# Amar-Aliaga/Stereo_Depth_Ruler

Measured on AMD Instinct MI355X. Metric: stereo Mpix/s (disparity+reproject) at 1280×720 d=128, 1/2/4/8 MI355X, higher is better.
Workload: dtype int16; 1 GPU; C2 (BASELINE configs[1]): 1280x720 d=128 MODE_SGBM 5-path + reprojectImageTo3D(Q, handleMissing), batch 1; width=1280, height=720, numDisparities=128, mode=MODE_SGBM, batch=1, pipeline=sgbm, parallelism=frame shard x1, streams_per_gpu=2

## Files before the change

stereo_depth_ruler_amd/csrc/sdr_device.hpp:

```cpp
#pragma once
#include <hip/hip_runtime.h>
#include <cfloat>
#include <stdint.h>

#include <type_traits>
#include <utility>

namespace sdr {

typedef short s16x2 __attribute__((ext_vector_type(2)));

constexpr int kMaxCost = 32767;
constexpr uint32_t kMaxPair = 0x7fff7fffu;

__device__ __forceinline__ s16x2 as_s16x2(uint32_t v) { return __builtin_bit_cast(s16x2, v); }
__device__ __forceinline__ uint32_t as_u32(s16x2 v) { return __builtin_bit_cast(uint32_t, v); }

__device__ __forceinline__ uint32_t pk_add(uint32_t a, uint32_t b) {
    return as_u32(as_s16x2(a) + as_s16x2(b));
}
__device__ __forceinline__ uint32_t pk_sub(uint32_t a, uint32_t b) {
    return as_u32(as_s16x2(a) - as_s16x2(b));
}
__device__ __forceinline__ uint32_t pk_add_sat(uint32_t a, uint32_t b) {
// ... 80 lines not shown
    uint32_t t = (uint32_t)__builtin_amdgcn_update_dpp((int)0xffffffff, (int)m, 0x142, 0xa, 0xf, false);
    m = min(m, t);
    t = (uint32_t)__builtin_amdgcn_update_dpp((int)0xffffffff, (int)m, 0x143, 0xc, 0xf, false);
    m = min(m, t);
    return (uint32_t)__builtin_amdgcn_readlane((int)m, 63);
}

__device__ __forceinline__ uint32_t row16_min_u32(uint32_t m) {
    m = min_u32_dpp<kDppQuadXor1>(m);
    m = min_u32_dpp<kDppQuadXor2>(m);
    m = min_u32_dpp<kDppRowHalfMirror>(m);
    return min_u32_dpp<kDppRowMirror>(m);
}

template <int K>
struct Regs {
    uint32_t r[K];
};

using Rsrc = __amdgpu_buffer_rsrc_t;
__device__ __forceinline__ Rsrc rsrc_at(const void* base) {
    return __builtin_amdgcn_make_buffer_rsrc(const_cast<void*>(base), (short)0, 0x7fffffff, 0x00020000);
}

template <int K, int AUX = 0>
__device__ __forceinline__ Regs<K> load_buf(Rsrc r, uint32_t vofs, uint32_t sofs = 0) {
    Regs<K> v;
    if constexpr (K == 1) {
        v.r[0] = __builtin_amdgcn_raw_buffer_load_b32(r, vofs, sofs, AUX);
    } else if constexpr (K == 2) {
        const auto t = __builtin_amdgcn_raw_buffer_load_b64(r, vofs, sofs, AUX);
        v.r[0] = t[0];
        v.r[1] = t[1];
    } else {
        static_assert(K % 4 == 0, "K = 1, 2 or a multiple of 4");
#pragma unroll
        for (int j = 0; j < K / 4; j++) {
            const auto t = __builtin_amdgcn_raw_buffer_load_b128(r, vofs + 16 * j, sofs, AUX);
            v.r[4 * j] = t[0]; v.r[4 * j + 1] = t[1]; v.r[4 * j + 2] = t[2]; v.r[4 * j + 3] = t[3];
        }
    }
    return v;
}

template <int K, int AUX = 2>
__device__ __forceinline__ void store_buf_nt(Rsrc r, uint32_t vofs, uint32_t sofs, const Regs<K>& v) {
    if constexpr (K == 1) {
        __builtin_amdgcn_raw_buffer_store_b32(v.r[0], r, vofs, sofs, AUX);
    } else if constexpr (K == 2) {
        __builtin_amdgcn_raw_buffer_store_b64((__attribute__((ext_vector_type(2))) uint32_t){v.r[0], v.r[1]}, r,
                                              vofs, sofs, AUX);
    } else {
#pragma unroll
        for (int j = 0; j < K / 4; j++)
            __builtin_amdgcn_raw_buffer_store_b128(
                (__attribute__((ext_vector_type(4))) uint32_t){v.r[4 * j], v.r[4 * j + 1], v.r[4 * j + 2],
                                                               v.r[4 * j + 3]},
                r, vofs + 16 * j, sofs, AUX);
    }
}

__device__ __forceinline__ int lane_id() { return (int)__lane_id(); }

inline int device_cus() {
    static int cache[64] = {};
    int dev = 0;
    (void)hipGetDevice(&dev);
    if (dev < 0 || dev >= 64) dev = 0;
    int cus = __atomic_load_n(&cache[dev], __ATOMIC_RELAXED);
    if (cus <= 0) {
        if (hipDeviceGetAttribute(&cus, hipDeviceAttributeMultiprocessorCount, dev) != hipSuccess || cus <= 0) cus = 256;
        __atomic_store_n(&cache[dev], cus, __ATOMIC_RELAXED);
    }
    return cus;
}

__device__ __forceinline__ int xcd_block(int h, int n) {
    const int q = n >> 3, r = n & 7, x = h & 7, k = h >> 3;
    return (x < r ? x * (q + 1) : r * (q + 1) + (x - r) * q) + k;
}

template <typename F, int... J>
__device__ __forceinline__ void unroll_rows(F& f, int k0, std::integer_sequence<int, J...>) {
    (f(k0 + J, std::integral_constant<int, J>{}), ...);
}
template <typename F, int... J>
__device__ __forceinline__ void unroll_rows_tail(F& f, int k0, int klast, std::integer_sequence<int, J...>) {
    ((k0 + J <= klast ? f(k0 + J, std::integral_constant<int, J>{}) : void()), ...);
}

__device__ __forceinline__ int div_trunc_small(int n, int d) {
    const int an = abs(n);
// ... 38 lines not shown
```

stereo_depth_ruler_amd/csrc/sdr_engine.hip:

```cpp
#include "../../include/sdr/sdr.h"
#include "sdr_internal.hpp"

#include <hip/hip_runtime.h>

#include <algorithm>
#include <cmath>
#include <cstdio>
#include <cstring>
#include <map>
#include <mutex>
#include <string>
#include <vector>

namespace {

thread_local std::string g_last_error;

int fail(int code, const std::string& msg) {
    g_last_error = msg;
    return code;
}

#define SDR_HIP(call)                                                                    \
    do {                                                                                 \
        hipError_t e_ = (call);                                                          \
        if (e_ != hipSuccess)                                                            \
            return fail(SDR_ERR_DEVICE, std::string(#call) + ": " + hipGetErrorString(e_)); \
    } while (0)

struct Eff {
    sdr::Geometry g;
    int mode, uniq, uniq_simd, disp12MaxDiff, ftzero, nstripes, invalid;
    int speckle_ws, speckle_diff, blockSize;
    int cost;
};

int make_eff(const sdr_sgbm_params& p, int W, int H, Eff* e, int cost = SDR_COST_BT) {
    if (cost != SDR_COST_BT && cost != SDR_COST_CENSUS_9X7) return fail(SDR_ERR_ARG, "unknown cost type");
    e->cost = cost;
    if (p.numDisparities <= 0 || p.numDisparities % 16 != 0)
// ... 267 lines not shown
    int drain() {
        for (const Out& o : outs) {
            SDR_HIP(hipEventSynchronize(ev[o.ev]));
            if (!o.dst) continue;
            if (o.dpitch == o.rowbytes) std::memcpy(o.dst, o.src, o.rowbytes * o.rows);
            else
                for (int r = 0; r < o.rows; r++) std::memcpy(o.dst + r * o.dpitch, o.src + r * o.rowbytes, o.rowbytes);
        }
        outs.clear();
        return SDR_OK;
    }
    void release() {
        for (auto e : ev) (void)hipEventDestroy(e);
        ev.clear();
        if (pin) (void)hipHostFree(pin);
        pin = nullptr;
        cap = 0;
    }
};
size_t stage_bytes(size_t n) { return (n + 255) & ~(size_t)255; }
}

struct sdr_sgbm {
    sdr_sgbm_params p{};
    int cost = SDR_COST_BT;
    size_t census_bytes = 0;
    int device = 0;
    hipStream_t stream = nullptr;
    hipStream_t own_stream = nullptr;
    Buf planesL, planesR, sink, C, Lr, Caux, draw, dlr, dfin, labels, sizes, mins, hin, hxyz, keys2;
    Buf sweep, status;
    int* status_host = nullptr;
    int sweep_spin = sdr::kSweepSpin;
    HostXfer hx;
    Buf cls_bgr, cls_gray, cls_small, cls_dl, cls_wls, cls_f, cls_conf, cls_filt;
    int timing = 0;
    hipEvent_t ev[4] = {nullptr, nullptr, nullptr, nullptr};
    std::vector<hipEvent_t> kev;
    std::vector<int> kkind;
    size_t kused = 0;
    size_t path_slack = 0, path_lslack = 0;
    hipStream_t side = nullptr;
    hipEvent_t fork = nullptr, join = nullptr;
    hipEvent_t done = nullptr;
    bool pending = false;
    bool persistent = true;
    bool relayed = false;
    bool needs_wait = false;
    int status_reported = 0;
    bool lr_skipped = false;
    sdr::Geometry lr_g{};
    int lr_frames = 0, lr_d12 = 0;
    size_t aux_slack = 0;
};

namespace {
constexpr unsigned kOrderEvent = hipEventDisableTiming | hipEventReleaseToDevice;
constexpr unsigned kTimerEvent = hipEventReleaseToDevice;
bool capturing(hipStream_t s) {
    hipStreamCaptureStatus cs = hipStreamCaptureStatusNone;
    return hipStreamIsCapturing(s, &cs) == hipSuccess && cs == hipStreamCaptureStatusActive;
}
hipError_t relay(sdr_sgbm* h, hipStream_t from) {
    hipError_t e = hipEventRecord(h->done, from);
    if (e == hipSuccess) e = hipStreamWaitEvent(h->own_stream, h->done, 0);
    if (e == hipSuccess) e = hipEventRecord(h->done, h->own_stream);
// ... 298 lines not shown
                d.Caux = Caux + s * (size_t)amax * g.W1 * g.D;
                d.aux_row0 = sp.s0;
                d.aux_rows = sp.aux_rows;
            }
        }
    } else if (e.mode == SDR_MODE_HH4) {
        add_dir(plS, sdr::DIR_S, nS, nullptr);
        add_dir(pls, sdr::DIR_N, nS, buf());
    } else if (sweep) {
    } else {
        add_dir(plS, sdr::DIR_S, nS, nullptr);
        if (e.mode == SDR_MODE_HH) add_dir(pls, sdr::DIR_N, nS, buf());
        add_dir(pls, sdr::DIR_SE, nD, buf());
        add_dir(pls, sdr::DIR_SW, nD, buf());
        if (e.mode == SDR_MODE_HH) {
            add_dir(pls, sdr::DIR_NE, nD, buf());
            add_dir(pls, sdr::DIR_NW, nD, buf());
        }
    }
    for (size_t s = 0; s < stripes.size(); s++) {
        const Stripe& sp = stripes[s];
        if (sp.aux_rows == 0 || sp.aux_rows != sp.end - sp.s0 || sp.out0 >= sp.end) continue;
        if (pls.nredir == sdr::kMaxCostAux) return fail(SDR_ERR_ARG, "too many 3WAY stripes");
        sdr::RowRedirect& r = pls.redir[pls.nredir++];
        r.lo = sp.out0;
        r.hi = sp.end;
        r.s0 = sp.s0;
        r.aux = Caux + s * (size_t)amax * g.W1 * g.D;
    }
    for (sdr::PathLaunch* pl : {&pls, &plS}) {
        pl->prefix[0] = 0;
        for (int i = 0; i < pl->ndirs; i++) pl->prefix[i + 1] = pl->prefix[i] + pl->d[i].nchains;
    }
    { KTimer kt(h, SDR_KERNEL_PATHS); sdr::launch_paths(g, pls, F, st); }
    if (sweep) {
        char* sb = (char*)h->sweep.p;
        SDR_HIP(hipMemsetAsync(sb, 0, sweep_flags + sizeof(int), st));
        sdr::SweepArgs sa{};
        sa.C = C;
        sa.cs_fstride = cells;
        sa.l_fstride = lfs;
        sa.l_pix = nrec * g.D;
        sa.flags = (int*)sb;
        sa.err = (int*)(sb + sweep_flags);
        sa.edge = (uint32_t*)(sb + sweep_flags + 256);
        sa.spin = h->sweep_spin;
        sdr::SweepWta sw{};
        sw.recs = Lr;
        sw.disp_raw = draw;
        sw.d2 = d2;
        sw.disp_fstride = px;
        sw.uniq = e.uniq;
        sw.uniq_simd = e.uniq_simd;
        std::lock_guard<std::mutex> lk(g_sweep_mu);
        hipEvent_t& last = g_sweep_last[h->device];
        if (last) SDR_HIP(hipStreamWaitEvent(st, last, 0));
        else SDR_HIP(hipEventCreateWithFlags(&last, kOrderEvent));
        for (int up = 1; up >= 0; up--) {
            sa.up = up;
            sa.ntiles = shp[up].ntiles;
            sa.nslots = shp[up].nslots;
            sa.rec = Lr + (size_t)2 * g.D;
            KTimer kt(h, up ? SDR_KERNEL_SWEEP : SDR_KERNEL_SWEEP_DOWN);
            sdr::launch_sweep(g, sa, sw, F, st);
            sa.flags += flags_n[up];
        }
// ... 52 lines not shown
    p->blockSize = 3;
    p->mode = SDR_MODE_SGBM;
    p->nstripes = 4;
}

void sdr_right_matcher_params(const sdr_sgbm_params* l, sdr_sgbm_params* r) {
    if (!l || !r) return;
    sdr_sgbm_params_default(r);
    r->minDisparity = -(l->minDisparity + l->numDisparities) + 1;
    r->numDisparities = l->numDisparities;
    r->blockSize = l->blockSize;
    r->uniquenessRatio = 0;
    r->P1 = l->P1;
    r->P2 = l->P2;
    r->mode = l->mode;
    r->preFilterCap = l->preFilterCap;
    r->disp12MaxDiff = 1000000;
    r->speckleWindowSize = 0;
    r->speckleRange = l->speckleRange;
    r->nstripes = l->nstripes;
    r->uniq_rule = l->uniq_rule;
}

int sdr_sgbm_create(const sdr_sgbm_params* p, int device, sdr_sgbm** out) {
    if (!p || !out) return fail(SDR_ERR_ARG, "null argument");
    *out = nullptr;
    int ndev = 0;
    SDR_HIP(hipGetDeviceCount(&ndev));
    if (device < 0 || device >= ndev) return fail(SDR_ERR_DEVICE, "invalid device index");
    SDR_HIP(hipSetDevice(device));
    sdr_sgbm* h = new sdr_sgbm();
    h->p = *p;
    h->device = device;
    if (hipStreamCreateWithFlags(&h->own_stream, hipStreamNonBlocking) != hipSuccess) {
        delete h;
        return fail(SDR_ERR_DEVICE, "hipStreamCreate failed");
    }
    h->stream = h->own_stream;
    for (auto& ev : h->ev) (void)hipEventCreateWithFlags(&ev, kTimerEvent);
    (void)hipEventCreateWithFlags(&h->done, kOrderEvent);
    *out = h;
    return SDR_OK;
}

int sdr_sgbm_destroy(sdr_sgbm* h) {
    if (!h) return SDR_OK;
    (void)hipSetDevice(h->device);
    if (h->stream && h->persistent) (void)hipStreamSynchronize(h->stream);
    if (h->own_stream && h->own_stream != h->stream) (void)hipStreamSynchronize(h->own_stream);
    if (h->status_host) (void)hipHostFree(h->status_host);
    for (Buf* b : {&h->sweep, &h->status, &h->planesL, &h->planesR, &h->sink, &h->C, &h->Lr, &h->Caux, &h->draw, &h->dlr, &h->dfin, &h->keys2,
                   &h->labels, &h->sizes, &h->mins, &h->hin, &h->hxyz, &h->cls_bgr,
                   &h->cls_gray, &h->cls_small, &h->cls_dl, &h->cls_wls, &h->cls_f,
                   &h->cls_conf, &h->cls_filt})
        if (b->p) (void)hipFree(b->p);
    h->hx.release();
    for (auto ev : h->ev)
        if (ev) (void)hipEventDestroy(ev);
    for (auto ev : h->kev) (void)hipEventDestroy(ev);
    if (h->side) (void)hipStreamSynchronize(h->side);
    if (h->fork) (void)hipEventDestroy(h->fork);
    if (h->join) (void)hipEventDestroy(h->join);
    if (h->done) (void)hipEventDestroy(h->done);
    if (h->side) (void)hipStreamDestroy(h->side);
    if (h->own_stream) (void)hipStreamDestroy(h->own_stream);
    delete h;
// ... 600 lines not shown
```

stereo_depth_ruler_amd/csrc/sdr_internal.hpp:

```cpp
#pragma once
#include <hip/hip_runtime.h>

#include "../../include/sdr/sdr.h"
#include <stddef.h>
#include <stdint.h>

#include <string>

namespace sdr {

constexpr int kMinSlots = 256;


struct Buf {
    void* p = nullptr;
    size_t n = 0;
};
int ensure(Buf& b, size_t bytes);
hipError_t scratch_alloc(void** p, size_t bytes, hipStream_t st);
hipError_t scratch_free(void* p, hipStream_t st);
int set_error(int code, const std::string& msg);

enum Dir : int {
    DIR_E = 0,
// ... 48 lines not shown
    int ylim;
    int hh_bottom;
    int TY;
    int16_t* sink;
    int naux;
    size_t aux_fstride;
    CostAux aux[kMaxCostAux];
};
size_t cost_sink_bytes(const Geometry& g);


constexpr int kMaxPathDirs = 24;
constexpr int kMaxPaths = 8;

struct PathDir {
    int dir;
    int nchains;
    int ybeg, yend, write_from;
    int aux_row0, aux_rows;
    const int16_t* Caux;
    int16_t* out;
};

struct RowRedirect {
    int lo, hi, s0;
    const int16_t* aux;
};

struct PathLaunch {
    const int16_t* C;
    size_t cs_fstride;
    size_t l_fstride;
    int l_pix;
    size_t aux_fstride;
    int ndirs;
    int prefix[kMaxPathDirs + 1];
    PathDir d[kMaxPathDirs];
    int nredir;
    RowRedirect redir[kMaxCostAux];
};

constexpr int kSweepOwn = 10;
constexpr int kSweepWaves = kSweepOwn + 2;
struct SweepArgs {
    const int16_t* C;
    size_t cs_fstride;
    int16_t* rec;
    size_t l_fstride;
    int l_pix;
    uint32_t* edge;
    int* flags;
    int* err;
    int ntiles, nslots;
    int up;
    int spin;
    int xcd;
};
struct SweepWta {
    const int16_t* recs;
    int16_t* disp_raw;
    uint32_t* d2;
    size_t disp_fstride;
    int uniq, uniq_simd;
};
constexpr int kSweepSpin = 1 << 20;
void launch_sweep_verdict(const int* err, int16_t* disp, size_t n, int F, int16_t invalid, int* mins,
                          int* sticky, hipStream_t st);
struct SweepShape {
    int cols, ntiles, nslots, npub, entry_words;
};
SweepShape sweep_shape(const Geometry& g, int F, bool up);
void launch_sweep(const Geometry& g, const SweepArgs& a, const SweepWta& w, int F, hipStream_t st);

constexpr int kSouthIdx = 2;
constexpr int kSouthPad = 64;
struct SouthWtaArgs {
    const int16_t* L;
    int npaths;
    int16_t* disp_raw;
    uint32_t* d2;
    size_t disp_fstride;
    int uniq, uniq_simd;
};
void launch_south_wta(const Geometry& g, const PathLaunch& pl, const SouthWtaArgs& a, int F,
                      hipStream_t st);

constexpr uint32_t kD2None = 0xffffffffu;
__device__ __forceinline__ int lr_at(const Geometry& g, const int16_t* __restrict__ raw,
                                     const uint32_t* __restrict__ d2, int x, int y, int d12) {
    const int invalid = (g.minD - 1) * 16;
    if (x < g.minX1 || x >= g.minX1 + g.W1) return invalid;
    const size_t ro = (size_t)y * g.W;
    const int d1 = raw[ro + x];
    if (d1 == invalid) return d1;
    const int _d = d1 >> 4, d_ = (d1 + 15) >> 4;
    const int _x = x - _d, x_ = x - d_;
    if (_x < 0 || _x >= g.W || x_ < 0 || x_ >= g.W) return d1;
    const uint32_t ka = d2[ro + _x], kb = d2[ro + x_];
    const int a2 = ka == kD2None ? invalid : (0xffff - (int)(ka & 0xffff)) + g.minX1 - _x;
    const int b2 = kb == kD2None ? invalid : (0xffff - (int)(kb & 0xffff)) + g.minX1 - x_;
    const bool bad = a2 >= g.minD && abs(a2 - _d) > d12 && b2 >= g.minD && abs(b2 - d_) > d12;
    return bad ? invalid : d1;
}
void launch_lr_apply(const Geometry& g, const int16_t* raw, const uint32_t* d2, int16_t* out,
                     size_t fstride, int disp12MaxDiff, int F, hipStream_t st);
struct LrSrc {
    Geometry g;
    const int16_t* raw;
    const uint32_t* d2;
    size_t fstride;
    int d12;
};

void launch_fill_s16(int16_t* p, int16_t v, size_t n, hipStream_t st);
void launch_prefilter(const uint8_t* L, const uint8_t* R, size_t stride, size_t fstride, int W,
                      int H, int F, int ftzero, const Planes& pl, hipStream_t st, int split = 1 << 30,
                      uint32_t* d2fill = nullptr);
bool cost_supported(const Geometry& g);
// ... 48 lines not shown
```

stereo_depth_ruler_amd/csrc/sdr_paths.hip:

```cpp
#include "sdr_device.hpp"
#include "sdr_internal.hpp"

#include <algorithm>

namespace sdr {

struct Chain {
    int x0, y0, dx, dy, len, kwrite;
};


__device__ __forceinline__ Chain make_chain(const Geometry& g, const PathDir& d, int c) {
    Chain ch;
    const int W1 = g.W1, H = g.H;
    ch.kwrite = 0;
    switch (d.dir) {
    case DIR_E: ch.x0 = 0; ch.y0 = c; ch.dx = 1; ch.dy = 0; ch.len = W1; break;
    case DIR_W: ch.x0 = W1 - 1; ch.y0 = c; ch.dx = -1; ch.dy = 0; ch.len = W1; break;
    case DIR_S:
        ch.x0 = c; ch.y0 = d.ybeg; ch.dx = 0; ch.dy = 1; ch.len = d.yend - d.ybeg;
        ch.kwrite = d.write_from - d.ybeg;
        break;
    case DIR_N: ch.x0 = c; ch.y0 = H - 1; ch.dx = 0; ch.dy = -1; ch.len = H; break;
    case DIR_SE:
        if (c < W1) { ch.x0 = c; ch.y0 = 0; } else { ch.x0 = 0; ch.y0 = c - W1 + 1; }
        ch.dx = 1; ch.dy = 1; ch.len = min(W1 - ch.x0, H - ch.y0);
        break;
    case DIR_SW:
        if (c < W1) { ch.x0 = c; ch.y0 = 0; } else { ch.x0 = W1 - 1; ch.y0 = c - W1 + 1; }
        ch.dx = -1; ch.dy = 1; ch.len = min(ch.x0 + 1, H - ch.y0);
        break;
    case DIR_NE:
        if (c < W1) { ch.x0 = c; ch.y0 = H - 1; } else { ch.x0 = 0; ch.y0 = H - 2 - (c - W1); }
        ch.dx = 1; ch.dy = -1; ch.len = min(W1 - ch.x0, ch.y0 + 1);
        break;
    default:
        if (c < W1) { ch.x0 = c; ch.y0 = H - 1; } else { ch.x0 = W1 - 1; ch.y0 = H - 2 - (c - W1); }
        ch.dx = -1; ch.dy = -1; ch.len = min(ch.x0 + 1, ch.y0 + 1);
        break;
    }
    return ch;
}

template <int K, bool PAD>
__device__ __forceinline__ void step_words(const Regs<K>& c, const Regs<K>& Lp, uint32_t delta2, uint32_t P1x2,
                                           bool active, uint32_t up, uint32_t dn, Regs<K>& L, uint32_t& m) {
    m = kMaxPair;
#pragma unroll
    for (int i = 0; i < K; i++) {
        const uint32_t dm1 = funnel16(Lp.r[i], i == 0 ? up : Lp.r[i == 0 ? 0 : i - 1]);
        const uint32_t dp1 = funnel16(i == K - 1 ? dn : Lp.r[i == K - 1 ? 0 : i + 1], Lp.r[i]);
        uint32_t t = pk_add_sat(pk_min(dm1, dp1), P1x2);
        t = pk_min(pk_min(t, Lp.r[i]), delta2);
        uint32_t l = pk_sub(pk_add(c.r[i], t), delta2);
        if constexpr (PAD) l = active ? l : kMaxPair;
        L.r[i] = l;
        m = pk_min(m, l);
    }
}

template <int K, bool PAD>
__device__ __forceinline__ Regs<K> path_step(Regs<K> c, Regs<K>& Lp, uint32_t& delta2, uint32_t P1x2,
                                             uint32_t P2x2, bool active, uint32_t& upr, uint32_t& dnr) {
    if constexpr (PAD) {
#pragma unroll
        for (int i = 0; i < K; i++) c.r[i] = active ? c.r[i] : kMaxPair;
    }
    const uint32_t up = upr = lane_from_prev(Lp.r[K - 1], upr);
    const uint32_t dn = dnr = lane_from_next(Lp.r[0], dnr);
    Regs<K> L;
    uint32_t m;
    step_words<K, PAD>(c, Lp, delta2, P1x2, active, up, dn, L, m);
    const uint32_t m16 = (uint32_t)__builtin_elementwise_min((unsigned short)(m & 0xffffu),
                                                              (unsigned short)(m >> 16));
    delta2 = wave_min_u32_uniform(m16) * 0x00010001u + P2x2;
    Lp = L;
    return L;
}

template <int DPL>
constexpr int paths_la() { return DPL == 8 ? 8 : 16; }
constexpr int kLoadNT = 2;

template <int DPL, bool PAD>
__global__ __launch_bounds__(256) void k_paths(Geometry g, PathLaunch pl) {
    constexpr int K = DPL / 2;
    constexpr int LA = paths_la<DPL>();
    constexpr int R = 2 * LA;
    const int lane = threadIdx.x & 63;
    const int cg = __builtin_amdgcn_readfirstlane(blockIdx.x * 4 + (threadIdx.x >> 6));
    const int f = blockIdx.y;
    if (cg >= pl.prefix[pl.ndirs]) return;
    int di = 0;
    while (cg >= pl.prefix[di + 1]) di++;
    const PathDir pd = pl.d[di];
    const Chain ch = make_chain(g, pd, cg - pl.prefix[di]);
    if (ch.len <= 0) return;

    const int D = g.D, W1 = g.W1;
    const bool active = !PAD || lane * DPL < D;
    const uint32_t lofs = (uint32_t)((PAD ? min(lane, D / DPL - 1) : lane) * DPL * 2);
    const ptrdiff_t rowb = (ptrdiff_t)(ch.dy * W1 + ch.dx) * D * 2;
    const ptrdiff_t rowl = (ptrdiff_t)(ch.dy * W1 + ch.dx) * pl.l_pix * 2;
    const char* cp = (const char*)(pl.C + (size_t)f * pl.cs_fstride + ((size_t)ch.y0 * W1 + ch.x0) * D);
    if (pd.dir == DIR_E || pd.dir == DIR_W) {
        for (int i = 0; i < pl.nredir; i++)
            if (ch.y0 >= pl.redir[i].lo && ch.y0 < pl.redir[i].hi)
                cp = (const char*)(pl.redir[i].aux + (size_t)f * pl.aux_fstride +
                                   ((size_t)(ch.y0 - pl.redir[i].s0) * W1 + ch.x0) * D);
    }
    char* op = (char*)(pd.out + (size_t)f * pl.l_fstride + ((size_t)ch.y0 * W1 + ch.x0) * pl.l_pix);
    const int last = ch.len - 1;
    const int low = rowb >= 0 ? 0 : last + LA;
    const Rsrc rC = rsrc_at(cp + (ptrdiff_t)low * rowb);
    uint32_t soff = (uint32_t)((ptrdiff_t)(0 - low) * rowb);
    Rsrc rO;
    uint32_t soffl = 0;
    auto rebase = [&](int k0) __attribute__((always_inline)) {
        const int lo = rowl >= 0 ? k0 : k0 + R - 1;
        rO = rsrc_at(op + (ptrdiff_t)lo * rowl);
        soffl = (uint32_t)((ptrdiff_t)(k0 - lo) * rowl);
    };

    Regs<K> cring[R];
#pragma unroll
    for (int j = 0; j < LA; j++) {
        cring[j] = load_buf<K>(rC, lofs, soff);
        soff += (uint32_t)rowb;
    }

    Regs<K> Lp;
#pragma unroll
    for (int i = 0; i < K; i++) Lp.r[i] = active ? 0u : kMaxPair;
    const uint32_t P1x2 = splat16(g.P1), P2x2 = splat16(g.P2);
    uint32_t delta2 = P2x2;
    uint32_t upr = kMaxPair, dnr = kMaxPair;

    const uint32_t sofs_st = active ? lofs : 0x80000000u;
    auto step = [&](const int, auto jc) __attribute__((always_inline)) {
        constexpr int j = decltype(jc)::value;
        const Regs<K> c = cring[j];
        cring[(j + LA) % R] = load_buf<K>(rC, lofs, soff);
        soff += (uint32_t)rowb;
        const Regs<K> L = path_step<K, PAD>(c, Lp, delta2, P1x2, P2x2, active, upr, dnr);
        store_buf_nt<K>(rO, sofs_st, soffl, L);
        soffl += (uint32_t)rowl;
        __builtin_amdgcn_sched_barrier(0);
    };
    int k0 = 0;
    for (; k0 + R <= ch.len; k0 += R) {
        rebase(k0);
        unroll_rows(step, k0, std::make_integer_sequence<int, R>{});
    }
    rebase(k0);
    unroll_rows_tail(step, k0, last, std::make_integer_sequence<int, R - 1>{});
}

template <bool PAD>
__device__ __forceinline__ Regs<2> path_step_tc(Regs<2> c, Regs<2>& Lp, uint32_t& delta2, uint32_t P1x2,
                                                uint32_t P2x2, bool active, uint32_t& upr, uint32_t& dnr,
                                                int lane) {
    constexpr int K = 2;
    if constexpr (PAD) {
#pragma unroll
        for (int i = 0; i < K; i++) c.r[i] = active ? c.r[i] : kMaxPair;
    }
    upr = lane_from_prev(Lp.r[K - 1], upr);
    dnr = lane_from_next(Lp.r[0], dnr);
    const uint32_t up = lane == 32 ? kMaxPair : upr;
    const uint32_t dn = lane == 31 ? kMaxPair : dnr;
    Regs<K> L;
    uint32_t m = kMaxPair;
#pragma unroll
    for (int i = 0; i < K; i++) {
        const uint32_t dm1 = funnel16(Lp.r[i], i == 0 ? up : Lp.r[i == 0 ? 0 : i - 1]);
        const uint32_t dp1 = funnel16(i == K - 1 ? dn : Lp.r[i == K - 1 ? 0 : i + 1], Lp.r[i]);
        uint32_t t = pk_add_sat(pk_min(dm1, dp1), P1x2);
        t = pk_min(pk_min(t, Lp.r[i]), delta2);
// ... 56 lines not shown
        soffl = (uint32_t)((ptrdiff_t)(k0 - lo) * rowl);
    };
    Regs<K> cring[R];
#pragma unroll
    for (int j = 0; j < LA; j++) {
        cring[j] = load_buf<K>(rC, vld, soff);
        soff += (uint32_t)rowb;
    }
    Regs<K> Lp;
#pragma unroll
    for (int i = 0; i < K; i++) Lp.r[i] = active ? 0u : kMaxPair;
    const uint32_t P1x2 = splat16(g.P1), P2x2 = splat16(g.P2);
    uint32_t delta2 = P2x2;
    uint32_t upr = kMaxPair, dnr = kMaxPair;
    auto step = [&](const int, auto jc) __attribute__((always_inline)) {
        constexpr int j = decltype(jc)::value;
        const Regs<K> c = cring[j];
        cring[(j + LA) % R] = load_buf<K>(rC, vld, soff);
        soff += (uint32_t)rowb;
        const Regs<K> L = path_step_tc<PAD>(c, Lp, delta2, P1x2, P2x2, active, upr, dnr, lane);
        store_buf_nt<K>(rO, vst, soffl, L);
        soffl += (uint32_t)rowl;
        __builtin_amdgcn_sched_barrier(0);
    };
    int k0 = 0;
    for (; k0 + R <= ch.len; k0 += R) {
        rebase(k0);
        unroll_rows(step, k0, std::make_integer_sequence<int, R>{});
    }
    rebase(k0);
    unroll_rows_tail(step, k0, last, std::make_integer_sequence<int, R - 1>{});
}

static bool paths_two_chain(const Geometry& g, const PathLaunch& pl, int F) {
    if (g.D > 128 || pl.nredir > 0) return false;
    for (int i = 0; i < pl.ndirs; i++)
        if (pl.d[i].dir != DIR_E && pl.d[i].dir != DIR_W && pl.d[i].dir != DIR_N) return false;
    return (long)pl.prefix[pl.ndirs] * F > 4L * device_cus();
}

void launch_paths(const Geometry& g, const PathLaunch& pl, int F, hipStream_t st) {
    const int total = pl.prefix[pl.ndirs];
    if (total <= 0) return;
    if (paths_two_chain(g, pl, F)) {
        int waves = 0;
        for (int i = 0; i < pl.ndirs; i++) waves += (pl.d[i].nchains + 1) / 2;
        const dim3 grid2((waves + 3) / 4, F);
        if (g.D < 128) hipLaunchKernelGGL((k_paths_tc<true>), grid2, dim3(256), 0, st, g, pl);
        else hipLaunchKernelGGL((k_paths_tc<false>), grid2, dim3(256), 0, st, g, pl);
        return;
    }
    dim3 grid((total + 3) / 4, F);
    if (g.D <= 128) {
        if (g.D < 128) hipLaunchKernelGGL((k_paths<2, true>), grid, dim3(256), 0, st, g, pl);
        else hipLaunchKernelGGL((k_paths<2, false>), grid, dim3(256), 0, st, g, pl);
    } else if (g.D <= 256) {
        if (g.D < 256) hipLaunchKernelGGL((k_paths<4, true>), grid, dim3(256), 0, st, g, pl);
        else hipLaunchKernelGGL((k_paths<4, false>), grid, dim3(256), 0, st, g, pl);
    } else {
        if (g.D < 512) hipLaunchKernelGGL((k_paths<8, true>), grid, dim3(256), 0, st, g, pl);
        else hipLaunchKernelGGL((k_paths<8, false>), grid, dim3(256), 0, st, g, pl);
    }
}

#ifndef SDR_SOUTH_CONS
#define SDR_SOUTH_CONS 3
#endif
#ifndef SDR_SOUTH_LAB
#define SDR_SOUTH_LAB 2
#endif
constexpr int kSouthConsumers = SDR_SOUTH_CONS;
constexpr int kSouthRPW = 4;
constexpr int kSouthRB = kSouthRPW * kSouthConsumers;
constexpr int kSouthLAB = SDR_SOUTH_LAB;
constexpr int kSouthSPad = 4;
constexpr int kStageBlocks = 32;
constexpr int kStageRows = kStageBlocks * kSouthRB;
constexpr uint32_t kNoWrite = 0xfffffffeu;
constexpr uint32_t kRejected = 0xffffffffu;

template <int DPL, bool PAD, int NP, bool TC = false>
__global__ __launch_bounds__(64 * (1 + kSouthConsumers)) void k_south_wta(Geometry g0, PathLaunch pl,
                                                                           SouthWtaArgs a) {
    static_assert(!TC || DPL == 2, "two columns per workgroup: the D <= 128 layout");
    const Geometry g = frame_geom(g0, blockIdx.y);
    constexpr int K = DPL / 2;
    constexpr int NCOL = TC ? 2 : 1;
    constexpr int PK = TC ? 2 : K;
    constexpr int RB = kSouthRB;
    constexpr int LAB = kSouthLAB;
    constexpr int LA = LAB * RB;
    constexpr int NS = LAB;
    constexpr int R = NS * RB;
    static_assert(LA + RB <= kSouthPad, "load overrun must fit the buffers' row slack");
    constexpr int WDPL = DPL * 4;
    constexpr int WK = WDPL / 2;
    constexpr int DMAX = 64 * DPL;
    constexpr int LSTR = DMAX / 2 + 4;
#ifndef SDR_SOUTH_TC_PD
#define SDR_SOUTH_TC_PD 2
#endif
    constexpr int PD = TC ? SDR_SOUTH_TC_PD : NP * WK * kSouthRPW <= 128 ? 2 : 1;
    static_assert((PD + 1) * RB <= kSouthPad, "consumer load overrun must fit the row slack");
    __shared__ uint32_t sL[2][RB][NCOL][LSTR];
    __shared__ uint32_t sS[kSouthConsumers][4][DMAX / 2 + kSouthSPad];
    __shared__ int16_t sRaw[2][NCOL][kStageRows];
    __shared__ uint32_t sKey[2][NCOL][kStageRows];
    const int lane = threadIdx.x & 63;
    const int wv = __builtin_amdgcn_readfirstlane(threadIdx.x >> 6);
    const int cg = blockIdx.x;
    const int f = blockIdx.y;
    int di = 0, c0i = 0;
    bool hasB = false;
    if constexpr (TC) {
        int w0 = 0;
        for (; di < pl.ndirs; di++) {
            const int nw = (pl.d[di].nchains + 1) / 2;
            if (cg < w0 + nw) break;
            w0 += nw;
        }
        if (di >= pl.ndirs) return;
        c0i = 2 * (cg - w0);
        hasB = c0i + 1 < pl.d[di].nchains;
    } else {
        while (cg >= pl.prefix[di + 1]) di++;
        c0i = cg - pl.prefix[di];
    }
    const PathDir pd = pl.d[di];
    const Chain ch = make_chain(g, pd, c0i);
    if (ch.len <= 0) return;
    const int D = g.D, W1 = g.W1;
    const size_t fofs = (size_t)f * pl.cs_fstride;
    const int last = ch.len - 1;
    const int nblk = (ch.len + RB - 1) / RB;

    if (wv == 0) {
        __builtin_amdgcn_s_setprio(2);
        const int half = TC ? lane >> 5 : 0, hl = TC ? lane & 31 : lane;
        constexpr int PDPL = 2 * PK;
        const bool active = (!TC || half == 0 || hasB) && (!PAD || hl * PDPL < D);
        const uint32_t lofs = (uint32_t)((PAD ? min(hl, D / PDPL - 1) : hl) * PDPL * 2) + (uint32_t)(half * D * 2);
        const ptrdiff_t rowb = (ptrdiff_t)W1 * D * 2;
        const int naux = pd.Caux ? pd.aux_rows : 0;
        const char* abase = pd.Caux ? (const char*)(pd.Caux + (size_t)f * pl.aux_fstride + (size_t)ch.x0 * D)
                                    : (const char*)pl.C;
        const char* c0 = (const char*)(pl.C + fofs + ((size_t)ch.y0 * W1 + ch.x0) * D);
        auto crow = [&](int k) { return c0 + (ptrdiff_t)min(k, last) * rowb; };
        Regs<PK> cring[R];
#pragma unroll
        for (int j = 0; j < LA; j++)
            cring[j] = load_buf<PK>(rsrc_at(j < naux ? abase + (ptrdiff_t)j * rowb : crow(j)), lofs);
        Regs<PK> Lp;
#pragma unroll
        for (int i = 0; i < PK; i++) Lp.r[i] = active ? 0u : kMaxPair;
        const uint32_t P1x2 = splat16(g.P1), P2x2 = splat16(g.P2);
        uint32_t delta2 = P2x2;
        uint32_t upr = kMaxPair, dnr = kMaxPair;
        auto block = [&](const int bb, auto ic) __attribute__((always_inline)) {
            uint32_t* dst = &sL[bb & 1][0][half][hl * PK];
            auto st = [&](const int, auto jc) __attribute__((always_inline)) {
                constexpr int j = decltype(jc)::value + decltype(ic)::value * RB;
                const Regs<PK> c = cring[j];
                cring[(j + LA) % R] = load_buf<PK, kLoadNT>(rsrc_at(crow(bb * RB + (j % RB) + LA)), lofs);
                Regs<PK> L;
                if constexpr (TC) L = path_step_tc<PAD>(c, Lp, delta2, P1x2, P2x2, active, upr, dnr, lane);
                else L = path_step<K, PAD>(c, Lp, delta2, P1x2, P2x2, active, upr, dnr);
#pragma unroll
                for (int i = 0; i < PK; i++) dst[(j % RB) * NCOL * LSTR + i] = L.r[i];
            };
            unroll_rows(st, bb * RB, std::make_integer_sequence<int, RB>{});
            __syncthreads();
        };
        int b = 0;
        for (; b + NS <= nblk; b += NS) unroll_rows(block, b, std::make_integer_sequence<int, NS>{});
        unroll_rows_tail(block, b, nblk - 1, std::make_integer_sequence<int, NS - 1>{});
        __syncthreads();
        return;
    }

    constexpr int RPASS = kSouthRPW / 4;
    constexpr int NPASS = NCOL * RPASS;
    const int gl = lane & 15, grp = lane >> 4;
    const bool wactive = !PAD || gl * WDPL < D;
    const int wd0 = (PAD ? min(gl, (D - 1) / WDPL) : gl) * WDPL;
    const ptrdiff_t bstepb = (ptrdiff_t)RB * W1 * pl.l_pix * 2;
    int rr[NPASS];
    uint32_t lofs[NPASS];
#pragma unroll
    for (int ps = 0; ps < NPASS; ps++) {
        const int col = ps / RPASS;
        rr[ps] = (wv - 1) * kSouthRPW + (ps % RPASS) * 4 + grp;
        lofs[ps] = (uint32_t)((((size_t)rr[ps] * W1 + col) * pl.l_pix + wd0) * 2);
    }
    const char* lbase = (const char*)(a.L + (size_t)f * pl.l_fstride + ((size_t)ch.y0 * W1 + ch.x0) * pl.l_pix);
    auto oload = [&](int q, int blk, int ps) __attribute__((always_inline)) {
        const bool need = blk * RB + RB > ch.kwrite;
        const Rsrc r = __builtin_amdgcn_make_buffer_rsrc(
            const_cast<char*>(lbase + (ptrdiff_t)min(blk, nblk - 1) * bstepb), (short)0, need ? 0x7fffffff : 0,
            0x00020000);
        return load_buf<WK, kLoadNT>(r, lofs[ps] + (uint32_t)(q * D * 2));
    };
    const int kw = ch.kwrite;
    const int invalid = (g.minD - 1) * 16;
    const bool check_uniq = a.uniq > 0 || !a.uniq_simd;
    const bool uniq_simd = a.uniq_simd != 0;
    const int lhs_scale = 100 - a.uniq;
    const double inv100u = 1.0 / (double)(100 - a.uniq) * (1.0 + 0x1p-40);
    const int x = ch.x0;
    int16_t* raw = a.disp_raw + (size_t)f * a.disp_fstride + x + g.minX1;
    uint32_t* d2 = a.d2 ? a.d2 + (size_t)f * a.disp_fstride : nullptr;
    const int x2base = x + g.minX1 - g.minD;

    auto flush = [&](int w) __attribute__((always_inline)) {
        const int r0 = w * kStageRows;
        const int n = min(kStageRows, ch.len - r0);
#pragma unroll
        for (int col = 0; col < NCOL; col++) {
            if (col > 0 && !hasB) break;
            for (int i = (wv - 1) * 64 + lane; i < n; i += 64 * kSouthConsumers) {
                const uint32_t key = sKey[w & 1][col][i];
                if (key == kNoWrite) continue;
                const size_t y = (size_t)(ch.y0 + r0 + i);
                raw[y * g.W + col] = sRaw[w & 1][col][i];
                if (d2 && key < kNoWrite) {
                    const int x2 = x2base + col - (int)(key & 0xffff);
                    if (x2 >= 0 && x2 < g.W)
                        atomicMin(&d2[y * g.W + x2], (key & 0xffff0000u) | (uint32_t)(0xffff - (x + col)));
                }
            }
        }
    };

    auto ssum = [&](const int b, const int r, const int col, const Regs<WK> (&o)[NP]) __attribute__((always_inline)) {
        const uint32_t* ls = &sL[b & 1][r][col][wd0 / 2];
        Regs<WK> St;
#pragma unroll
        for (int i = 0; i < WK; i++) {
            uint32_t acc = 0;
#pragma unroll
            for (int p = 0; p <= NP; p++) {
                const uint32_t v = p == kSouthIdx ? ls[i] : o[p < kSouthIdx ? p : p - 1].r[i];
                acc = p == 0 ? v : pk_add_sat(acc, v);
            }
            if constexpr (PAD && DPL == 8) acc = wd0 + 2 * i < D ? acc : kMaxPair;
            St.r[i] = acc;
        }
        return St;
    };
    auto rows = [&](const int b, const int r, const int col, const Regs<WK>& St) __attribute__((always_inline)) {
        const int k = b * RB + r;
        const bool rowok = k >= kw && k <= last;
        uint32_t key = 0xffffffffu;
#pragma unroll
        for (int i = 0; i < WK; i++) {
            const uint32_t d = (uint32_t)(gl * WDPL + 2 * i);
            const uint32_t lo = (uint32_t)((int)(short)(St.r[i] & 0xffff) + 32768);
            const uint32_t hi = (uint32_t)((int)(short)(St.r[i] >> 16) + 32768);
            key = min(key, min((lo << 16) | d, (hi << 16) | (d + 1)));
        }
        uint32_t* srow = &sS[wv - 1][grp][0];
#pragma unroll
        for (int i = 0; i < WK; i++) ((uint32_t __attribute__((may_alias))*)srow)[gl * WK + i] = St.r[i];
        key = row16_min_u32(wactive ? key : 0xffffffffu);
        const int minS = (int)(key >> 16) - 32768;
        const int best = (int)(key & 0xffff);
        const int dm = max(best - 1, 0), dp = min(best + 1, D - 1);
        typedef int16_t __attribute__((may_alias)) s16a;
        typedef uint32_t __attribute__((may_alias)) u32a;
        s16a* s16 = (s16a*)srow;
        const int Sm = s16[dm];
        const int Sp = s16[dp];
        s16[dm] = 0x7fff;
        s16[best] = 0x7fff;
        s16[dp] = 0x7fff;
        uint32_t m2 = kMaxPair;
#pragma unroll
        for (int i = 0; i < WK; i++) m2 = pk_min(m2, ((u32a*)srow)[gl * WK + i]);
        m2 = wactive ? m2 : kMaxPair;
        m2 = pk_min(m2, funnel16(m2, m2));
        m2 = row16_min_u32(m2);
        const int min2 = (int)(m2 & 0x7fff);
        const int thr16 = (int)(short)((int)((double)(100 * minS) * inv100u) + 1);
        const bool reject = check_uniq && (uniq_simd ? (min2 < thr16) : (min2 * lhs_scale < minS * 100));
        if (gl == 0 && k <= last) {
            int out = invalid;
            uint32_t okey = kNoWrite;
            if (rowok) {
                okey = kRejected;
                if (!reject && minS < kMaxCost) {
                    const int den = max(Sm + Sp - 2 * minS, 1);
                    const int qq = div_trunc_small((Sm - Sp) * 16 + den, 2 * den);
                    out = best * 16 + (((0 < best) & (best < D - 1)) ? qq : 0) + g.minD * 16;
                    okey = ((uint32_t)minS << 16) | (uint32_t)best;
                }
            }
            sRaw[(k / kStageRows) & 1][col][k % kStageRows] = (int16_t)out;
            sKey[(k / kStageRows) & 1][col][k % kStageRows] = okey;
        }
    };

    Regs<WK> oring[PD][NPASS][NP];
#pragma unroll
    for (int s = 0; s < PD; s++)
#pragma unroll
        for (int ps = 0; ps < NPASS; ps++)
#pragma unroll
            for (int q = 0; q < NP; q++) oring[s][ps][q] = oload(q, s, ps);

    auto consume_sync = [&](const int b, auto sc) __attribute__((always_inline)) {
        constexpr int s = decltype(sc)::value;
#pragma unroll
        for (int ps = 0; ps < NPASS; ps++) {
            const Regs<WK> St = ssum(b, rr[ps], ps / RPASS, oring[s][ps]);
#pragma unroll
            for (int q = 0; q < NP; q++) oring[s][ps][q] = oload(q, b + PD, ps);
            if (ps < RPASS || hasB) rows(b, rr[ps], ps / RPASS, St);
        }
        __syncthreads();
        if (b % kStageBlocks == kStageBlocks - 1 || b == nblk - 1) flush(b / kStageBlocks);
    };
    __syncthreads();
    int b = 0;
    for (; b + PD <= nblk; b += PD) unroll_rows(consume_sync, b, std::make_integer_sequence<int, PD>{});
    unroll_rows_tail(consume_sync, b, nblk - 1, std::make_integer_sequence<int, PD>{});
}

__global__ __launch_bounds__(256) void k_lr_apply(Geometry g0, const int16_t* __restrict__ raw,
                                                  const uint32_t* __restrict__ d2,
                                                  int16_t* __restrict__ out, size_t fstride, int d12) {
    const Geometry g = frame_geom(g0, blockIdx.y);
    const int y = blockIdx.x, f = blockIdx.y;
    const size_t fo = (size_t)f * fstride;
    for (int x = threadIdx.x; x < g.W; x += 256)
        out[fo + (size_t)y * g.W + x] = (int16_t)lr_at(g, raw + fo, d2 + fo, x, y, d12);
}

template <int DPL, bool PAD>
static void launch_south_np(const Geometry& g, const PathLaunch& pl, const SouthWtaArgs& a, int F,
                            hipStream_t st) {
    dim3 grid(pl.prefix[pl.ndirs], F);
    dim3 block(64 * (1 + kSouthConsumers));
    if constexpr (DPL == 2) {
        const int cus = device_cus();
        if (a.npaths <= 5 && (long)pl.prefix[pl.ndirs] * F > 8L * cus) {
            int wgs = 0;
            for (int i = 0; i < pl.ndirs; i++) wgs += (pl.d[i].nchains + 1) / 2;
            const dim3 grid2(wgs, F);
            switch (a.npaths) {
            case 3: hipLaunchKernelGGL((k_south_wta<2, PAD, 2, true>), grid2, block, 0, st, g, pl, a); return;
            case 4: hipLaunchKernelGGL((k_south_wta<2, PAD, 3, true>), grid2, block, 0, st, g, pl, a); return;
            default: hipLaunchKernelGGL((k_south_wta<2, PAD, 4, true>), grid2, block, 0, st, g, pl, a); return;
            }
        }
    }
    switch (a.npaths) {
    case 3: hipLaunchKernelGGL((k_south_wta<DPL, PAD, 2>), grid, block, 0, st, g, pl, a); break;
    case 4: hipLaunchKernelGGL((k_south_wta<DPL, PAD, 3>), grid, block, 0, st, g, pl, a); break;
    case 5: hipLaunchKernelGGL((k_south_wta<DPL, PAD, 4>), grid, block, 0, st, g, pl, a); break;
    default: hipLaunchKernelGGL((k_south_wta<DPL, PAD, 7>), grid, block, 0, st, g, pl, a); break;
    }
}

void launch_south_wta(const Geometry& g, const PathLaunch& pl, const SouthWtaArgs& a, int F,
                      hipStream_t st) {
    if (pl.prefix[pl.ndirs] <= 0) return;
    if (g.D <= 128) {
        if (g.D < 128) launch_south_np<2, true>(g, pl, a, F, st);
        else launch_south_np<2, false>(g, pl, a, F, st);
    } else if (g.D <= 256) {
        if (g.D < 256) launch_south_np<4, true>(g, pl, a, F, st);
        else launch_south_np<4, false>(g, pl, a, F, st);
    } else {
        if (g.D < 512) launch_south_np<8, true>(g, pl, a, F, st);
        else launch_south_np<8, false>(g, pl, a, F, st);
    }
}

// ... 7 lines not shown
```

Before: 1637 Mpix/s.

## Store non-south path costs as packed 12-bit records relative to cost

For D=128 the path kernels now store a 12-bit excess value E = delta2 - t per disparity instead of the full 16-bit path cost L, packed into three dwords per four-lane group using a quad DPP broadcast. The south WTA kernel loads these 96-bit records, unpacks them and rebuilds L as (cost + t - delta2) from the matching-cost row, which it now also keeps in shared memory. This cuts path-record traffic to three quarters of its previous size. In exchange it adds pack/unpack ALU work and extra LDS use, and it relies on P2 fitting in 12 bits. An SDR_PATH_REC=16 environment variable restores the old 16-bit records.

```diff
diff --git a/stereo_depth_ruler_amd/csrc/sdr_device.hpp b/stereo_depth_ruler_amd/csrc/sdr_device.hpp
--- a/stereo_depth_ruler_amd/csrc/sdr_device.hpp
+++ b/stereo_depth_ruler_amd/csrc/sdr_device.hpp
@@ -136,6 +136,11 @@
         const auto t = __builtin_amdgcn_raw_buffer_load_b64(r, vofs, sofs, AUX);
         v.r[0] = t[0];
         v.r[1] = t[1];
+    } else if constexpr (K == 3) {
+        const auto t = __builtin_amdgcn_raw_buffer_load_b96(r, vofs, sofs, AUX);
+        v.r[0] = t[0];
+        v.r[1] = t[1];
+        v.r[2] = t[2];
     } else {
         static_assert(K % 4 == 0, "K = 1, 2 or a multiple of 4");
 #pragma unroll
@@ -162,6 +167,19 @@
                                                                v.r[4 * j + 3]},
                 r, vofs + 16 * j, sofs, AUX);
     }
+}
+
+constexpr int kDppQuadLane3 = 0xFF;
+__device__ __forceinline__ uint32_t rec12_pack(uint32_t p, int lane) {
+    const uint32_t p3 = dpp_mov<kDppQuadLane3>(p);
+    return p | (((p3 >> (4 * (lane & 3))) & 0x000f000fu) << 12);
+}
+__device__ __forceinline__ Regs<4> rec12_unpack(const Regs<3>& w) {
+    Regs<4> p;
+#pragma unroll
+    for (int j = 0; j < 3; j++) p.r[j] = w.r[j] & 0x0fff0fffu;
+    p.r[3] = ((w.r[0] >> 12) & 0x000f000fu) | ((w.r[1] >> 8) & 0x00f000f0u) | ((w.r[2] >> 4) & 0x0f000f00u);
+    return p;
 }
 
 __device__ __forceinline__ int lane_id() { return (int)__lane_id(); }
diff --git a/stereo_depth_ruler_amd/csrc/sdr_engine.hip b/stereo_depth_ruler_amd/csrc/sdr_engine.hip
--- a/stereo_depth_ruler_amd/csrc/sdr_engine.hip
+++ b/stereo_depth_ruler_amd/csrc/sdr_engine.hip
@@ -6,6 +6,7 @@
 #include <algorithm>
 #include <cmath>
 #include <cstdio>
+#include <cstdlib>
 #include <cstring>
 #include <map>
 #include <mutex>
@@ -339,6 +340,7 @@
     Buf sweep, status;
     int* status_host = nullptr;
     int sweep_spin = sdr::kSweepSpin;
+    bool rec16 = false;
     HostXfer hx;
     Buf cls_bgr, cls_gray, cls_small, cls_dl, cls_wls, cls_f, cls_conf, cls_filt;
     int timing = 0;
@@ -703,6 +705,15 @@
         pl->prefix[0] = 0;
         for (int i = 0; i < pl->ndirs; i++) pl->prefix[i + 1] = pl->prefix[i] + pl->d[i].nchains;
     }
+    const bool rec12 = !h->rec16 && !sweep && g.P2 >= 0 && g.P2 <= 4095 &&
+                       (e.mode == SDR_MODE_SGBM || e.mode == SDR_MODE_HH || e.mode == SDR_MODE_HH4) &&
+                       sdr::path_rec12_supported(g, pls, plS, nrec + 1, F);
+    if (rec12) {
+        const int recel = g.D * 3 / 4;
+        pls.rec12 = plS.rec12 = 1;
+        pls.l_pix = plS.l_pix = nrec * recel;
+        for (int i = 0; i < pls.ndirs; i++) pls.d[i].out = Lr + (size_t)i * recel;
+    }
     { KTimer kt(h, SDR_KERNEL_PATHS); sdr::launch_paths(g, pls, F, st); }
     if (sweep) {
         char* sb = (char*)h->sweep.p;
@@ -821,6 +832,8 @@
     sdr_sgbm* h = new sdr_sgbm();
     h->p = *p;
     h->device = device;
+    const char* rec = getenv("SDR_PATH_REC");
+    h->rec16 = rec && atoi(rec) == 16;
     if (hipStreamCreateWithFlags(&h->own_stream, hipStreamNonBlocking) != hipSuccess) {
         delete h;
         return fail(SDR_ERR_DEVICE, "hipStreamCreate failed");
diff --git a/stereo_depth_ruler_amd/csrc/sdr_internal.hpp b/stereo_depth_ruler_amd/csrc/sdr_internal.hpp
--- a/stereo_depth_ruler_amd/csrc/sdr_internal.hpp
+++ b/stereo_depth_ruler_amd/csrc/sdr_internal.hpp
@@ -104,6 +104,7 @@
     size_t cs_fstride;
     size_t l_fstride;
     int l_pix;
+    int rec12;
     size_t aux_fstride;
     int ndirs;
     int prefix[kMaxPathDirs + 1];
@@ -156,6 +157,9 @@
 };
 void launch_south_wta(const Geometry& g, const PathLaunch& pl, const SouthWtaArgs& a, int F,
                       hipStream_t st);
+bool paths_two_chain(const Geometry& g, const PathLaunch& pl, int F);
+bool south_two_col(const Geometry& g, const PathLaunch& pl, int npaths, int F);
+bool path_rec12_supported(const Geometry& g, const PathLaunch& pls, const PathLaunch& plS, int npaths, int F);
 
 constexpr uint32_t kD2None = 0xffffffffu;
 __device__ __forceinline__ int lr_at(const Geometry& g, const int16_t* __restrict__ raw,
diff --git a/stereo_depth_ruler_amd/csrc/sdr_paths.hip b/stereo_depth_ruler_amd/csrc/sdr_paths.hip
--- a/stereo_depth_ruler_amd/csrc/sdr_paths.hip
+++ b/stereo_depth_ruler_amd/csrc/sdr_paths.hip
@@ -42,9 +42,10 @@
     return ch;
 }
 
-template <int K, bool PAD>
+template <int K, bool PAD, bool WE = false>
 __device__ __forceinline__ void step_words(const Regs<K>& c, const Regs<K>& Lp, uint32_t delta2, uint32_t P1x2,
-                                           bool active, uint32_t up, uint32_t dn, Regs<K>& L, uint32_t& m) {
+                                           bool active, uint32_t up, uint32_t dn, Regs<K>& L, uint32_t& m,
+                                           Regs<K>* E = nullptr) {
     m = kMaxPair;
 #pragma unroll
     for (int i = 0; i < K; i++) {
@@ -54,14 +55,16 @@
         t = pk_min(pk_min(t, Lp.r[i]), delta2);
         uint32_t l = pk_sub(pk_add(c.r[i], t), delta2);
         if constexpr (PAD) l = active ? l : kMaxPair;
+        if constexpr (WE) E->r[i] = pk_sub(delta2, t);
         L.r[i] = l;
         m = pk_min(m, l);
     }
 }
 
-template <int K, bool PAD>
+template <int K, bool PAD, bool WE = false>
 __device__ __forceinline__ Regs<K> path_step(Regs<K> c, Regs<K>& Lp, uint32_t& delta2, uint32_t P1x2,
-                                             uint32_t P2x2, bool active, uint32_t& upr, uint32_t& dnr) {
+                                             uint32_t P2x2, bool active, uint32_t& upr, uint32_t& dnr,
+                                             Regs<K>* E = nullptr) {
     if constexpr (PAD) {
 #pragma unroll
         for (int i = 0; i < K; i++) c.r[i] = active ? c.r[i] : kMaxPair;
@@ -70,7 +73,7 @@
     const uint32_t dn = dnr = lane_from_next(Lp.r[0], dnr);
     Regs<K> L;
     uint32_t m;
-    step_words<K, PAD>(c, Lp, delta2, P1x2, active, up, dn, L, m);
+    step_words<K, PAD, WE>(c, Lp, delta2, P1x2, active, up, dn, L, m, E);
     const uint32_t m16 = (uint32_t)__builtin_elementwise_min((unsigned short)(m & 0xffffu),
                                                               (unsigned short)(m >> 16));
     delta2 = wave_min_u32_uniform(m16) * 0x00010001u + P2x2;
@@ -82,8 +85,9 @@
 constexpr int paths_la() { return DPL == 8 ? 8 : 16; }
 constexpr int kLoadNT = 2;
 
-template <int DPL, bool PAD>
+template <int DPL, bool PAD, bool R12 = false>
 __global__ __launch_bounds__(256) void k_paths(Geometry g, PathLaunch pl) {
+    static_assert(!R12 || (DPL == 2 && !PAD), "12-bit records: D = 128");
     constexpr int K = DPL / 2;
     constexpr int LA = paths_la<DPL>();
     constexpr int R = 2 * LA;
@@ -136,14 +140,22 @@
     uint32_t delta2 = P2x2;
     uint32_t upr = kMaxPair, dnr = kMaxPair;
 
-    const uint32_t sofs_st = active ? lofs : 0x80000000u;
+    const uint32_t sofs_st = R12 ? ((lane & 3) == 3 ? 0x80000000u : (uint32_t)((lane >> 2) * 12 + (lane & 3) * 4))
+                                 : active ? lofs : 0x80000000u;
     auto step = [&](const int, auto jc) __attribute__((always_inline)) {
         constexpr int j = decltype(jc)::value;
         const Regs<K> c = cring[j];
         cring[(j + LA) % R] = load_buf<K>(rC, lofs, soff);
         soff += (uint32_t)rowb;
-        const Regs<K> L = path_step<K, PAD>(c, Lp, delta2, P1x2, P2x2, active, upr, dnr);
-        store_buf_nt<K>(rO, sofs_st, soffl, L);
+        if constexpr (R12) {
+            Regs<K> E;
+            (void)path_step<K, PAD, true>(c, Lp, delta2, P1x2, P2x2, active, upr, dnr, &E);
+            E.r[0] = rec12_pack(E.r[0], lane);
+            store_buf_nt<K>(rO, sofs_st, soffl, E);
+        } else {
+            const Regs<K> L = path_step<K, PAD>(c, Lp, delta2, P1x2, P2x2, active, upr, dnr);
+            store_buf_nt<K>(rO, sofs_st, soffl, L);
+        }
         soffl += (uint32_t)rowl;
         __builtin_amdgcn_sched_barrier(0);
     };
@@ -266,7 +278,7 @@
     unroll_rows_tail(step, k0, last, std::make_integer_sequence<int, R - 1>{});
 }
 
-static bool paths_two_chain(const Geometry& g, const PathLaunch& pl, int F) {
+bool paths_two_chain(const Geometry& g, const PathLaunch& pl, int F) {
     if (g.D > 128 || pl.nredir > 0) return false;
     for (int i = 0; i < pl.ndirs; i++)
         if (pl.d[i].dir != DIR_E && pl.d[i].dir != DIR_W && pl.d[i].dir != DIR_N) return false;
@@ -287,6 +299,7 @@
     dim3 grid((total + 3) / 4, F);
     if (g.D <= 128) {
         if (g.D < 128) hipLaunchKernelGGL((k_paths<2, true>), grid, dim3(256), 0, st, g, pl);
+        else if (pl.rec12) hipLaunchKernelGGL((k_paths<2, false, true>), grid, dim3(256), 0, st, g, pl);
         else hipLaunchKernelGGL((k_paths<2, false>), grid, dim3(256), 0, st, g, pl);
     } else if (g.D <= 256) {
         if (g.D < 256) hipLaunchKernelGGL((k_paths<4, true>), grid, dim3(256), 0, st, g, pl);
@@ -313,10 +326,14 @@
 constexpr uint32_t kNoWrite = 0xfffffffeu;
 constexpr uint32_t kRejected = 0xffffffffu;
 
-template <int DPL, bool PAD, int NP, bool TC = false>
+template <int DPL, bool PAD, int NP, bool TC = false, bool R12 = false>
 __global__ __launch_bounds__(64 * (1 + kSouthConsumers)) void k_south_wta(Geometry g0, PathLaunch pl,
                                                                            SouthWtaArgs a) {
     static_assert(!TC || DPL == 2, "two columns per workgroup: the D <= 128 layout");
+    static_assert(!R12 || (DPL == 2 && !PAD && !TC), "12-bit records: D = 128, one column");
+    constexpr int NPL = R12 ? 2 : 1;
+    constexpr int WR = R12 ? 3 : DPL * 2;
+    constexpr int RECB = 64 * DPL * (R12 ? 3 : 4) / 2;
     const Geometry g = frame_geom(g0, blockIdx.y);
     constexpr int K = DPL / 2;
     constexpr int NCOL = TC ? 2 : 1;
@@ -336,7 +353,7 @@
 #endif
     constexpr int PD = TC ? SDR_SOUTH_TC_PD : NP * WK * kSouthRPW <= 128 ? 2 : 1;
     static_assert((PD + 1) * RB <= kSouthPad, "consumer load overrun must fit the row slack");
-    __shared__ uint32_t sL[2][RB][NCOL][LSTR];
+    __shared__ uint32_t sL[2][RB][NCOL][NPL][LSTR];
     __shared__ uint32_t sS[kSouthConsumers][4][DMAX / 2 + kSouthSPad];
     __shared__ int16_t sRaw[2][NCOL][kStageRows];
     __shared__ uint32_t sKey[2][NCOL][kStageRows];
@@ -391,7 +408,7 @@
         uint32_t delta2 = P2x2;
         uint32_t upr = kMaxPair, dnr = kMaxPair;
         auto block = [&](const int bb, auto ic) __attribute__((always_inline)) {
-            uint32_t* dst = &sL[bb & 1][0][half][hl * PK];
+            uint32_t* dst = &sL[bb & 1][0][half][0][hl * PK];
             auto st = [&](const int, auto jc) __attribute__((always_inline)) {
                 constexpr int j = decltype(jc)::value + decltype(ic)::value * RB;
                 const Regs<PK> c = cring[j];
@@ -400,7 +417,10 @@
                 if constexpr (TC) L = path_step_tc<PAD>(c, Lp, delta2, P1x2, P2x2, active, upr, dnr, lane);
                 else L = path_step<K, PAD>(c, Lp, delta2, P1x2, P2x2, active, upr, dnr);
 #pragma unroll
-                for (int i = 0; i < PK; i++) dst[(j % RB) * NCOL * LSTR + i] = L.r[i];
+                for (int i = 0; i < PK; i++) {
+                    dst[(j % RB) * NCOL * NPL * LSTR + i] = L.r[i];
+                    if constexpr (R12) dst[(j % RB) * NCOL * NPL * LSTR + LSTR + i] = c.r[i];
+                }
             };
             unroll_rows(st, bb * RB, std::make_integer_sequence<int, RB>{});
             __syncthreads();
@@ -424,7 +444,7 @@
     for (int ps = 0; ps < NPASS; ps++) {
         const int col = ps / RPASS;
         rr[ps] = (wv - 1) * kSouthRPW + (ps % RPASS) * 4 + grp;
-        lofs[ps] = (uint32_t)((((size_t)rr[ps] * W1 + col) * pl.l_pix + wd0) * 2);
+        lofs[ps] = (uint32_t)(((size_t)rr[ps] * W1 + col) * pl.l_pix * 2 + (R12 ? gl * 12 : wd0 * 2));
     }
     const char* lbase = (const char*)(a.L + (size_t)f * pl.l_fstride + ((size_t)ch.y0 * W1 + ch.x0) * pl.l_pix);
     auto oload = [&](int q, int blk, int ps) __attribute__((always_inline)) {
@@ -432,7 +452,7 @@
         const Rsrc r = __builtin_amdgcn_make_buffer_rsrc(
             const_cast<char*>(lbase + (ptrdiff_t)min(blk, nblk - 1) * bstepb), (short)0, need ? 0x7fffffff : 0,
             0x00020000);
-        return load_buf<WK, kLoadNT>(r, lofs[ps] + (uint32_t)(q * D * 2));
+        return load_buf<WR, kLoadNT>(r, lofs[ps] + (uint32_t)(R12 ? q * RECB : q * D * 2));
     };
     const int kw = ch.kwrite;
     const int invalid = (g.minD - 1) * 16;
@@ -465,15 +485,27 @@
         }
     };
 
-    auto ssum = [&](const int b, const int r, const int col, const Regs<WK> (&o)[NP]) __attribute__((always_inline)) {
-        const uint32_t* ls = &sL[b & 1][r][col][wd0 / 2];
+    auto ssum = [&](const int b, const int r, const int col, const Regs<WR> (&o)[NP]) __attribute__((always_inline)) {
+        const uint32_t* ls = &sL[b & 1][r][col][0][wd0 / 2];
+        Regs<WK> Lq[NP];
+#pragma unroll
+        for (int q = 0; q < NP; q++) {
+            if constexpr (R12) {
+                const Regs<4> e = rec12_unpack(o[q]);
+#pragma unroll
+                for (int i = 0; i < WK; i++) Lq[q].r[i] = pk_sub(ls[LSTR + i], e.r[i]);
+            } else {
+#pragma unroll
+                for (int i = 0; i < WK; i++) Lq[q].r[i] = o[q].r[i];
+            }
+        }
         Regs<WK> St;
 #pragma unroll
         for (int i = 0; i < WK; i++) {
             uint32_t acc = 0;
 #pragma unroll
             for (int p = 0; p <= NP; p++) {
-                const uint32_t v = p == kSouthIdx ? ls[i] : o[p < kSouthIdx ? p : p - 1].r[i];
+                const uint32_t v = p == kSouthIdx ? ls[i] : Lq[p < kSouthIdx ? p : p - 1].r[i];
                 acc = p == 0 ? v : pk_add_sat(acc, v);
             }
             if constexpr (PAD && DPL == 8) acc = wd0 + 2 * i < D ? acc : kMaxPair;
@@ -533,7 +565,7 @@
         }
     };
 
-    Regs<WK> oring[PD][NPASS][NP];
+    Regs<WR> oring[PD][NPASS][NP];
 #pragma unroll
     for (int s = 0; s < PD; s++)
 #pragma unroll
@@ -569,14 +601,31 @@
         out[fo + (size_t)y * g.W + x] = (int16_t)lr_at(g, raw + fo, d2 + fo, x, y, d12);
 }
 
+bool south_two_col(const Geometry& g, const PathLaunch& pl, int npaths, int F) {
+    return g.D <= 128 && npaths <= 5 && (long)pl.prefix[pl.ndirs] * F > 8L * device_cus();
+}
+
+bool path_rec12_supported(const Geometry& g, const PathLaunch& pls, const PathLaunch& plS, int npaths, int F) {
+    return g.D == 128 && (npaths == 4 || npaths == 5 || npaths == 8) && pls.nredir == 0 &&
+           !paths_two_chain(g, pls, F) && !south_two_col(g, plS, npaths, F);
+}
+
 template <int DPL, bool PAD>
 static void launch_south_np(const Geometry& g, const PathLaunch& pl, const SouthWtaArgs& a, int F,
                             hipStream_t st) {
     dim3 grid(pl.prefix[pl.ndirs], F);
     dim3 block(64 * (1 + kSouthConsumers));
+    if constexpr (DPL == 2 && !PAD) {
+        if (pl.rec12) {
+            switch (a.npaths) {
+            case 4: hipLaunchKernelGGL((k_south_wta<2, false, 3, false, true>), grid, block, 0, st, g, pl, a); return;
+            case 5: hipLaunchKernelGGL((k_south_wta<2, false, 4, false, true>), grid, block, 0, st, g, pl, a); return;
+            default: hipLaunchKernelGGL((k_south_wta<2, false, 7, false, true>), grid, block, 0, st, g, pl, a); return;
+            }
+        }
+    }
     if constexpr (DPL == 2) {
-        const int cus = device_cus();
-        if (a.npaths <= 5 && (long)pl.prefix[pl.ndirs] * F > 8L * cus) {
+        if (south_two_col(g, pl, a.npaths, F)) {
             int wgs = 0;
             for (int i = 0; i < pl.ndirs; i++) wgs += (pl.d[i].nchains + 1) / 2;
             const dim3 grid2(wgs, F);
```

Result: faster. 1692 Mpix/s (median of 6 runs) (+3.4%).
